# tczhangzhi/pytorch-distributed

Measured on NVIDIA H100. Metric: ResNet-50 images/sec (device-timed, max over ranks), higher is better.
Workload: dtype bf16; 1 GPU; model=resnet50, global_batch=256, image_size=224, parallelism=dp1, entry=distributed, comm=fused, nvls=False, channels_last=True, fused_bn=True, optimizer=fused, cuda_graph=True, l2_policy=inputs larger than L2 (4 x 38.5 MB bf16 batches + GBs of activations per step), overlap_optimizer=True, bucket_view=False, cudnn=deterministic

## Files before the change

### pytorch_distributed_b200/csrc/bindings.cpp

```cpp
#include <torch/extension.h>

#include "hvd_core.h"
#include "host.h"
#include "symm.h"

namespace py = pybind11;
using namespace ptd;

namespace {

at::Tensor arena_view(const std::shared_ptr<SymmArena>& a, int64_t rank, int64_t offset_bytes, int64_t numel, const std::string& dtype) {
  at::ScalarType st;
  if (dtype == "float32") st = at::kFloat;
  else if (dtype == "bfloat16") st = at::kBFloat16;
  else if (dtype == "float16") st = at::kHalf;
  else if (dtype == "int32") st = at::kInt;
  else if (dtype == "uint8") st = at::kByte;
  else throw std::runtime_error("unsupported arena view dtype " + dtype);
  const int64_t esz = (int64_t)c10::elementSize(st);
  TORCH_CHECK(offset_bytes >= 0 && offset_bytes + numel * esz <= a->bytes(), "arena view out of range");
  TORCH_CHECK(offset_bytes % esz == 0, "misaligned arena view");
  const int r = a->single_process() ? (int)rank : a->rank();
  void* p = reinterpret_cast<void*>(a->ptr(r) + offset_bytes);
  auto keep = a;
// ... 69 lines not shown
        launch_ll_allreduce(a->ctx(channel), in, out, scale, a->ll_seq_ptr());
      })
      .def("sync_bn",
           [](std::shared_ptr<SymmArena> a, int channel, int64_t xoff, int64_t calls_ptr, int as_rank) {
             TORCH_CHECK(xoff >= 0 && xoff % 16 == 0 && xoff + kSyncBnAreaBytes <= a->bytes(), "sync BN exchange area outside the arena");
             TORCH_CHECK(calls_ptr != 0, "sync BN call counters missing");
             return SyncBN{a->ctx(channel, as_rank), xoff, reinterpret_cast<uint32_t*>(calls_ptr)};
           },
           py::arg("channel"), py::arg("xoff"), py::arg("calls_ptr"), py::arg("as_rank") = 0);

  m.def("pack_pointers", &pack_pointers);
  m.def("fused_sgd_flat", &fused_sgd_flat, py::arg("grad"), py::arg("master"), py::arg("momentum"), py::arg("model_copy"), py::arg("hyper"),
        py::arg("found_inf"), py::arg("nesterov"), py::arg("first_step"));
  m.def("fused_sgd_multi", &fused_sgd_multi);
  m.def("multi_tensor_scale", &multi_tensor_scale);
  m.def("multi_tensor_axpby", &multi_tensor_axpby);
  m.def("amp_update_scale", &amp_update_scale);
  const auto sync_arg = py::arg("sync") = static_cast<const SyncBN*>(nullptr);
  m.def("bn_act_forward", &bn_act_forward, py::arg("x"), py::arg("residual"), py::arg("weight"), py::arg("bias"), py::arg("running_mean"),
        py::arg("running_var"), py::arg("num_batches_tracked"), py::arg("training"), py::arg("momentum"), py::arg("eps"), py::arg("relu"),
        py::arg("need_mask"), py::arg("work"), py::arg("stats_ready"), sync_arg);
  m.def("bn_act_backward", &bn_act_backward, py::arg("dy"), py::arg("x"), py::arg("mask"), py::arg("weight"), py::arg("saved"), py::arg("relu"),
        py::arg("has_residual"), py::arg("work"), sync_arg);
  m.def("bn_act_backward2", &bn_act_backward2, py::arg("dy_a"), py::arg("dy_b"), py::arg("x"), py::arg("mask"), py::arg("weight"),
        py::arg("saved"), py::arg("relu"), py::arg("work"), sync_arg);
  m.def("stem_forward", &stem_forward, py::arg("x"), py::arg("weight"), py::arg("bias"), py::arg("running_mean"), py::arg("running_var"),
        py::arg("num_batches_tracked"), py::arg("training"), py::arg("momentum"), py::arg("eps"), py::arg("need_code"), py::arg("work"), sync_arg);
  m.def("stem_forward_pre", &stem_forward_pre, py::arg("x"), py::arg("weight"), py::arg("bias"), py::arg("running_mean"), py::arg("running_var"),
        py::arg("num_batches_tracked"), py::arg("training"), py::arg("momentum"), py::arg("eps"), py::arg("need_code"), py::arg("work"), sync_arg);
  m.def("stem_backward", &stem_backward, py::arg("dp"), py::arg("x"), py::arg("code"), py::arg("weight"), py::arg("saved"), py::arg("work"),
        sync_arg);
  m.def("stem_im2col", &stem_im2col);
  m.def("conv1x1_bnstats", &conv1x1_bnstats, py::arg("x"), py::arg("weight"), py::arg("gsum"), sync_arg);
  m.def("normalize_nhwc", &normalize_nhwc);
  m.def("resample_normalize", &resample_normalize, py::arg("arena"), py::arg("n"), py::arg("out_h"), py::arg("out_w"), py::arg("max_rows"),
        py::arg("a"), py::arg("b"), py::arg("out_dtype"), py::arg("channels_last"));
  m.def("p2p_copy_multi", &p2p_copy_multi);

  py::class_<FusionQueue, std::shared_ptr<FusionQueue>>(m, "FusionQueue")
      .def(py::init<int64_t, double, int64_t>(), py::arg("fusion_threshold_bytes"), py::arg("cycle_time_ms"), py::arg("cycle_bytes") = 0)
      .def("wait_idle", &FusionQueue::wait_idle, py::arg("timeout_ms"), py::call_guard<py::gil_scoped_release>())
      .def("wake", &FusionQueue::wake)
      .def("set_cycle_bytes", &FusionQueue::set_cycle_bytes)
      .def("cycle_bytes", &FusionQueue::cycle_bytes)
      .def("enable_timeline", &FusionQueue::enable_timeline)
      .def("timeline", &FusionQueue::timeline)
      .def("enqueue", &FusionQueue::enqueue, py::arg("name"), py::arg("nbytes"), py::arg("order_key"))
      .def("next_group", &FusionQueue::next_group, py::arg("timeout_ms"), py::call_guard<py::gil_scoped_release>())
      .def("flush", &FusionQueue::flush)
      .def("mark_done", &FusionQueue::mark_done)
      .def("wait", &FusionQueue::wait, py::arg("handle"), py::arg("timeout_ms"), py::call_guard<py::gil_scoped_release>())
      .def("pending", &FusionQueue::pending)
      .def("shutdown", &FusionQueue::shutdown)
      .def("stats", &FusionQueue::stats);
}
```

### pytorch_distributed_b200/csrc/bn_act.cu

```cuda
#include <ATen/cuda/CUDAContext.h>
#include <c10/cuda/CUDAGuard.h>
#include <torch/extension.h>

#include <map>

#include "bn_combine.cuh"
#include "common.cuh"
#include "host.h"

namespace ptd {

constexpr int kBnThreads = 256;
constexpr int kBnWarps = kBnThreads / 32;

struct RowMap {
  int cgs;
  int tpr;
  int rpp;
  int rlocal;
  int cg0;
  bool active;
  bool pow2;
};
__device__ __forceinline__ RowMap row_map(int C) {
// ... 600 lines not shown
          float dz = to_f32<T>(from_f32<T>(d[k] + e[k]));
          if constexpr (RELU) dz = (bits >> k) & 1u ? dz : 0.f;
          d[k] = dz;
          s[k] += dz;
          q[k] += dz * (v[k] - mean[k]);
        }
        store8<T>(gout + r * C + coff, d);
      }
#pragma unroll
      for (int k = 0; k < 8; ++k) q[k] *= saved[C + cg * 8 + k];
    }
    cta_combine(m, cgb, s, q, sm, part, C);
  }
}

template <typename T>
static void bwd2_impl(const at::Tensor& dya, const at::Tensor& dyb, const at::Tensor& mask, const at::Tensor& x, const at::Tensor& saved,
                      at::Tensor& work, const at::Tensor& w, at::Tensor& g_out, at::Tensor& dx, at::Tensor& dw, at::Tensor& db, bool relu,
                      const SyncBN* sync) {
  const Geometry g = geometry(x);
  cudaStream_t st = at::cuda::getCurrentCUDAStream();
  T* gp = reinterpret_cast<T*>(g_out.data_ptr());
  const auto reduce = relu ? bn_bwd_reduce_sum_kernel<T, true> : bn_bwd_reduce_sum_kernel<T, false>;
  int rpb;
  const int rgrid = reduce_grid(g, &rpb, resident_ctas(reduce, g.smem));
  at::Tensor part = partials(x, rgrid, g.C);
  reduce<<<rgrid, kBnThreads, g.smem, st>>>(reinterpret_cast<const T*>(dya.data_ptr()), reinterpret_cast<const T*>(dyb.data_ptr()),
                                            relu ? mask.data_ptr<uint8_t>() : nullptr, reinterpret_cast<const T*>(x.data_ptr()),
                                            saved.data_ptr<float>(), gp, part.data_ptr<float>(), g.M, g.C, rpb);
  C10_CUDA_KERNEL_LAUNCH_CHECK();
  bwd_apply<T>(g, part, gp, nullptr, x, saved, work, w, dx, nullptr, dw, db, false, sync, st);
}

std::vector<at::Tensor> bn_act_backward2(const at::Tensor& dy_a_in, const at::Tensor& dy_b_in, const at::Tensor& x,
                                         const c10::optional<at::Tensor>& mask_opt, const at::Tensor& weight, const at::Tensor& saved,
                                         bool relu, at::Tensor work, const SyncBN* sync) {
  check_nhwc(x, "x");
  const auto cl = at::MemoryFormat::ChannelsLast;
  at::Tensor dya = dy_a_in.is_contiguous(cl) ? dy_a_in : dy_a_in.contiguous(cl);
  at::Tensor dyb = dy_b_in.is_contiguous(cl) ? dy_b_in : dy_b_in.contiguous(cl);
  TORCH_CHECK(dya.scalar_type() == x.scalar_type() && dya.sizes() == x.sizes() && dya.device() == x.device(), "dy_a must match x");
  TORCH_CHECK(dyb.scalar_type() == x.scalar_type() && dyb.sizes() == x.sizes() && dyb.device() == x.device(), "dy_b must match x");
  at::Tensor mask;
  if (relu) {
    TORCH_CHECK(mask_opt.has_value() && mask_opt->defined() && mask_opt->scalar_type() == at::kByte && mask_opt->numel() == x.numel() / 8,
                "ReLU backward needs the forward's bit mask");
    mask = *mask_opt;
  }
  const int C = (int)x.size(1);
  check_work(work, C, sync);
  TORCH_CHECK(saved.defined() && saved.scalar_type() == at::kFloat && saved.numel() >= 2 * C, "saved statistics missing");
  c10::cuda::CUDAGuard guard(x.device());
  at::Tensor g = at::empty_like(x, x.options().memory_format(cl));
  at::Tensor dx = at::empty_like(x, x.options().memory_format(cl));
  at::Tensor dw = at::empty_like(weight), db = at::empty_like(weight);
  for_act_dtype(x, [&](auto t) { bwd2_impl<typename decltype(t)::type>(dya, dyb, mask, x, saved, work, weight, g, dx, dw, db, relu, sync); });
  return {dx, g, dw, db};
}

}

namespace ptd {

struct PoolGeom { int H, W, OH, OW; };

__device__ __forceinline__ void stem_scale_shift(const float* gsum, const float* rm, const float* rv, const void* w, const void* b, int wdt,
// ... 433 lines not shown
```

### pytorch_distributed_b200/csrc/gemm_bnstats.cu

```cuda
#include <ATen/cuda/CUDAContext.h>
#include <c10/cuda/CUDAGuard.h>
#include <cuda.h>
#include <torch/extension.h>

#include "common.cuh"
#include "host.h"

namespace ptd {

constexpr int kBlockM = 128;
constexpr int kBlockK = 64;
constexpr int kConsumerThreads = 256;
constexpr int kGemmThreads = kConsumerThreads + 32;

template <int BLOCK_N> struct GemmCfg {
  static constexpr int kStages = BLOCK_N == 256 ? 3 : 4;
  static constexpr int kABytes = kBlockM * kBlockK * 2;
  static constexpr int kBBytes = BLOCK_N * kBlockK * 2;
  static constexpr int kCBytes = kBlockM * BLOCK_N * 2;
  static constexpr int kStatFloats = 2 * 4 * 128;
  static constexpr int kSmem = 1024 + kStages * (kABytes + kBBytes) + kCBytes + kStatFloats * 4 + 2 * kStages * 8;
};

__device__ __forceinline__ uint32_t smem_u32(const void* p) { return (uint32_t)__cvta_generic_to_shared(p); }
// ... 37 lines not shown
      "wgmma.mma_async.sync.aligned.m64n64k16.f32." TY "." TY " "                                                     \
      "{%0, %1, %2, %3, %4, %5, %6, %7, %8, %9, %10, %11, %12, %13, %14, %15, "                                       \
      "%16, %17, %18, %19, %20, %21, %22, %23, %24, %25, %26, %27, %28, %29, %30, %31}, %32, %33, p, 1, 1, 0, 0;\n\t}" \
      : PTD_F8(0), PTD_F8(8), PTD_F8(16), PTD_F8(24)                                                                  \
      : "l"(adesc), "l"(bdesc), "r"(accumulate))
#define PTD_WGMMA_N128(TY)                                                                                            \
  asm volatile(                                                                                                       \
      "{\n\t.reg .pred p;\n\tsetp.ne.b32 p, %66, 0;\n\t"                                                              \
      "wgmma.mma_async.sync.aligned.m64n128k16.f32." TY "." TY " "                                                    \
      "{%0, %1, %2, %3, %4, %5, %6, %7, %8, %9, %10, %11, %12, %13, %14, %15, "                                       \
      "%16, %17, %18, %19, %20, %21, %22, %23, %24, %25, %26, %27, %28, %29, %30, %31, "                              \
      "%32, %33, %34, %35, %36, %37, %38, %39, %40, %41, %42, %43, %44, %45, %46, %47, "                              \
      "%48, %49, %50, %51, %52, %53, %54, %55, %56, %57, %58, %59, %60, %61, %62, %63}, %64, %65, p, 1, 1, 0, 0;\n\t}" \
      : PTD_F8(0), PTD_F8(8), PTD_F8(16), PTD_F8(24), PTD_F8(32), PTD_F8(40), PTD_F8(48), PTD_F8(56)                  \
      : "l"(adesc), "l"(bdesc), "r"(accumulate))

template <typename T> __device__ __forceinline__ void wgmma_n64(float* d, uint64_t adesc, uint64_t bdesc, int accumulate) {
  if constexpr (std::is_same<T, __half>::value) PTD_WGMMA_N64("f16");
  else PTD_WGMMA_N64("bf16");
}
template <typename T> __device__ __forceinline__ void wgmma_n128(float* d, uint64_t adesc, uint64_t bdesc, int accumulate) {
  if constexpr (std::is_same<T, __half>::value) PTD_WGMMA_N128("f16");
  else PTD_WGMMA_N128("bf16");
}
#undef PTD_WGMMA_N64
#undef PTD_WGMMA_N128
#undef PTD_F8

template <int N> __device__ __forceinline__ void fence_regs(float (&d)[N]) {
#pragma unroll
  for (int i = 0; i < N; ++i) asm volatile("" : "+f"(d[i])::"memory");
}

template <typename T, int BLOCK_N>
__global__ void __launch_bounds__(kGemmThreads, 1) gemm_bnstats_kernel(const __grid_constant__ CUtensorMap tmap_a,
                                                                       const __grid_constant__ CUtensorMap tmap_b,
                                                                       const __grid_constant__ CUtensorMap tmap_c,
                                                                       float* __restrict__ part, int N, int K, int m_tiles,
                                                                       int n_tiles, int ctas_per_n) {
  using Cfg = GemmCfg<BLOCK_N>;
  constexpr int kStages = Cfg::kStages;
  constexpr int kInstN = BLOCK_N >= 128 ? 128 : 64;
  constexpr int kBoxes = BLOCK_N / 64;
  extern __shared__ uint8_t smem_raw[];
  uint8_t* smem = reinterpret_cast<uint8_t*>((reinterpret_cast<uintptr_t>(smem_raw) + 1023) & ~(uintptr_t)1023);
  uint8_t* smem_a = smem;
  uint8_t* smem_b = smem_a + kStages * Cfg::kABytes;
  uint8_t* smem_c = smem_b + kStages * Cfg::kBBytes;
  float* smem_stats = reinterpret_cast<float*>(smem_c + Cfg::kCBytes);
  uint64_t* full_bar = reinterpret_cast<uint64_t*>(smem_stats + Cfg::kStatFloats);
  uint64_t* empty_bar = full_bar + kStages;

  const int warp = threadIdx.x >> 5, lane = threadIdx.x & 31;
  const int n_tile = blockIdx.x % n_tiles;
  const int m_first = blockIdx.x / n_tiles;
  const int n0 = n_tile * BLOCK_N;
  const int num_kb = K / kBlockK;

  if (threadIdx.x == 0) {
    for (int s = 0; s < kStages; ++s) { mbar_init(&full_bar[s], 1); mbar_init(&empty_bar[s], kConsumerThreads / 32); }
    asm volatile("fence.mbarrier_init.release.cluster;" ::: "memory");
  }
  __syncthreads();

  if (warp == kConsumerThreads / 32) {
    if (lane == 0) {
      asm volatile("prefetch.tensormap [%0];" ::"l"(&tmap_a) : "memory");
      asm volatile("prefetch.tensormap [%0];" ::"l"(&tmap_b) : "memory");
      uint32_t it = 0;
      for (int mt = m_first; mt < m_tiles; mt += ctas_per_n) {
        for (int kb = 0; kb < num_kb; ++kb, ++it) {
          const int s = it % kStages;
          mbar_wait(&empty_bar[s], ((it / kStages) & 1) ^ 1);
          mbar_expect_tx(&full_bar[s], Cfg::kABytes + Cfg::kBBytes);
          tma_load_2d(smem_a + s * Cfg::kABytes, &tmap_a, &full_bar[s], kb * kBlockK, mt * kBlockM);
          tma_load_2d(smem_b + s * Cfg::kBBytes, &tmap_b, &full_bar[s], kb * kBlockK, n0);
        }
      }
    }
    return;
  }

  const int wg = warp >> 2, t = threadIdx.x & 127, w = warp & 3;
  uint8_t* stg = smem_c + wg * (Cfg::kCBytes / 2);
  float acc[BLOCK_N / 2] = {};
  const int r0 = 16 * w + (lane >> 2);
  constexpr int kPairs = BLOCK_N / 2, kParts = 128 / kPairs, kRows = 64 / kParts;
  const int p = t % kPairs, rpart = t / kPairs;
  const int p_box = p >> 5, p_gran = (p & 31) >> 2, p_byte = (p & 3) * 4;
  float s0 = 0.f, s1 = 0.f, q0 = 0.f, q1 = 0.f;

  uint32_t it = 0;
  for (int mt = m_first; mt < m_tiles; mt += ctas_per_n) {
    for (int kb = 0; kb < num_kb; ++kb, ++it) {
      const int s = it % kStages;
      mbar_wait(&full_bar[s], (it / kStages) & 1);
      const uint64_t adesc = gmma_desc(smem_a + s * Cfg::kABytes + wg * 64 * 128);
      const uint64_t bdesc = gmma_desc(smem_b + s * Cfg::kBBytes);
      fence_regs(acc);
      asm volatile("wgmma.fence.sync.aligned;" ::: "memory");
#pragma unroll
      for (int k = 0; k < kBlockK / 16; ++k) {
#pragma unroll
        for (int h = 0; h < BLOCK_N / kInstN; ++h) {
          if constexpr (kInstN == 128) wgmma_n128<T>(acc + h * 64, adesc + 2 * k, bdesc + h * 8 * kInstN + 2 * k, (kb | k) != 0);
          else wgmma_n64<T>(acc + h * 32, adesc + 2 * k, bdesc + h * 8 * kInstN + 2 * k, (kb | k) != 0);
        }
      }
      asm volatile("wgmma.commit_group.sync.aligned;" ::: "memory");
      asm volatile("wgmma.wait_group.sync.aligned 0;" ::: "memory");
      fence_regs(acc);
      if (lane == 0) mbar_arrive(&empty_bar[s]);
    }

    if (t == 0) asm volatile("cp.async.bulk.wait_group.read 0;" ::: "memory");
    named_barrier(1 + wg, 128);
#pragma unroll
    for (int j = 0; j < BLOCK_N / 8; ++j) {
      uint8_t* box = stg + (j >> 3) * 8192 + (lane & 3) * 4;
      const int g = j & 7;
      *reinterpret_cast<uint32_t*>(box + r0 * 128 + ((g ^ (r0 & 7)) << 4)) = Wire<T>::pack2(acc[4 * j], acc[4 * j + 1]);
      *reinterpret_cast<uint32_t*>(box + (r0 + 8) * 128 + ((g ^ (r0 & 7)) << 4)) =
          Wire<T>::pack2(acc[4 * j + 2], acc[4 * j + 3]);
    }
    asm volatile("fence.proxy.async.shared::cta;" ::: "memory");
    named_barrier(1 + wg, 128);
    if (t == 0) {
#pragma unroll
      for (int b = 0; b < kBoxes; ++b)
        asm volatile("cp.async.bulk.tensor.2d.global.shared::cta.bulk_group [%0, {%2, %3}], [%1];"
                     ::"l"(&tmap_c), "r"(smem_u32(stg + b * 8192)), "r"(n0 + b * 64), "r"(mt * kBlockM + wg * 64) : "memory");
      asm volatile("cp.async.bulk.commit_group;" ::: "memory");
    }
    const uint8_t* src = stg + p_box * 8192 + p_byte;
#pragma unroll 8
    for (int r = rpart * kRows; r < rpart * kRows + kRows; ++r) {
      const float2 f = Wire<T>::unpack2(*reinterpret_cast<const uint32_t*>(src + r * 128 + ((p_gran ^ (r & 7)) << 4)));
      s0 += f.x; q0 += f.x * f.x;
      s1 += f.y; q1 += f.y * f.y;
    }
  }
  if (t == 0) asm volatile("cp.async.bulk.wait_group 0;" ::: "memory");
  float* my = smem_stats + wg * 4 * 128 + t;
  my[0] = s0; my[128] = s1; my[256] = q0; my[384] = q1;
  named_barrier(3, kConsumerThreads);
  for (int i = threadIdx.x; i < 2 * BLOCK_N; i += kConsumerThreads) {
    const int half = i >= BLOCK_N, col = i - half * BLOCK_N;
    const int pair = col >> 1, which = half * 2 + (col & 1);
    float v = 0.f;
    for (int w2 = 0; w2 < 2; ++w2)
      for (int pt = 0; pt < kParts; ++pt) v += smem_stats[w2 * 4 * 128 + which * 128 + pt * kPairs + pair];
    part[(size_t)m_first * 2 * N + half * N + n0 + col] = v;
  }
}

typedef CUresult (*EncodeTiledFn)(CUtensorMap*, CUtensorMapDataType, cuuint32_t, void*, const cuuint64_t*, const cuuint64_t*, const cuuint32_t*,
                                  const cuuint32_t*, CUtensorMapInterleave, CUtensorMapSwizzle, CUtensorMapL2promotion, CUtensorMapFloatOOBfill);

static EncodeTiledFn encode_fn() {
  static EncodeTiledFn fn = nullptr;
  if (!fn) {
    void* p = nullptr;
    cudaDriverEntryPointQueryResult q;
    TORCH_CHECK(cudaGetDriverEntryPoint("cuTensorMapEncodeTiled", &p, cudaEnableDefault, &q) == cudaSuccess && p, "cuTensorMapEncodeTiled not found");
    fn = reinterpret_cast<EncodeTiledFn>(p);
  }
  return fn;
}

static CUtensorMap make_map(CUtensorMapDataType dtype, const void* ptr, int64_t rows, int64_t cols, int box_rows,
                            CUtensorMapL2promotion promo) {
  CUtensorMap m;
  cuuint64_t dims[2] = {(cuuint64_t)cols, (cuuint64_t)rows};
  cuuint64_t strides[1] = {(cuuint64_t)cols * 2};
  cuuint32_t box[2] = {(cuuint32_t)kBlockK, (cuuint32_t)box_rows};
  cuuint32_t estr[2] = {1, 1};
  CUresult r = encode_fn()(&m, dtype, 2, const_cast<void*>(ptr), dims, strides, box, estr, CU_TENSOR_MAP_INTERLEAVE_NONE,
                           CU_TENSOR_MAP_SWIZZLE_128B, promo, CU_TENSOR_MAP_FLOAT_OOB_FILL_NONE);
  TORCH_CHECK(r == CUDA_SUCCESS, "cuTensorMapEncodeTiled failed: ", (int)r);
  return m;
}

template <typename T, int BLOCK_N>
static void launch_gemm(const at::Tensor& a, const at::Tensor& b, at::Tensor& c, at::Tensor& gsum, int M, int N, int K, const SyncBN* sync) {
  constexpr int smem = GemmCfg<BLOCK_N>::kSmem;
  static bool configured[64] = {};
  const int dev = a.get_device();
  if (!configured[dev & 63]) {
    C10_CUDA_CHECK(cudaFuncSetAttribute(gemm_bnstats_kernel<T, BLOCK_N>, cudaFuncAttributeMaxDynamicSharedMemorySize, smem));
    configured[dev & 63] = true;
  }
  constexpr CUtensorMapDataType dt = std::is_same<T, __half>::value ? CU_TENSOR_MAP_DATA_TYPE_FLOAT16 : CU_TENSOR_MAP_DATA_TYPE_BFLOAT16;
  const CUtensorMap ma = make_map(dt, a.data_ptr(), M, K, kBlockM, CU_TENSOR_MAP_L2_PROMOTION_L2_256B);
  const CUtensorMap mb = make_map(dt, b.data_ptr(), N, K, BLOCK_N, CU_TENSOR_MAP_L2_PROMOTION_L2_256B);
  const CUtensorMap mc = make_map(dt, c.data_ptr(), M, N, 64, CU_TENSOR_MAP_L2_PROMOTION_NONE);
  const int m_tiles = (M + kBlockM - 1) / kBlockM, n_tiles = N / BLOCK_N;
  const int sms = at::cuda::getCurrentDeviceProperties()->multiProcessorCount;
  const int ctas_per_n = std::max(1, std::min(m_tiles, sms / n_tiles));
  const int grid = ctas_per_n * n_tiles;
  cudaStream_t st = at::cuda::getCurrentCUDAStream();
  at::Tensor part = at::empty({ctas_per_n, 2 * N}, gsum.options());
  gemm_bnstats_kernel<T, BLOCK_N><<<grid, kGemmThreads, smem, st>>>(ma, mb, mc, part.data_ptr<float>(), N, K, m_tiles, n_tiles, ctas_per_n);
  C10_CUDA_KERNEL_LAUNCH_CHECK();
  finish_sums(part.data_ptr<float>(), ctas_per_n, N, M, gsum.data_ptr<float>(), sync, st);
}

template <typename T>
static void launch_gemm_for(const at::Tensor& a, const at::Tensor& b, at::Tensor& c, at::Tensor& gsum, int M, int N, int K, const SyncBN* sync) {
  static const int max_bn = getenv("PTD_GEMM_BLOCK_N") ? atoi(getenv("PTD_GEMM_BLOCK_N")) : 256;
  if (N % 256 == 0 && max_bn >= 256) launch_gemm<T, 256>(a, b, c, gsum, M, N, K, sync);
  else if (N % 128 == 0 && max_bn >= 128) launch_gemm<T, 128>(a, b, c, gsum, M, N, K, sync);
  else launch_gemm<T, 64>(a, b, c, gsum, M, N, K, sync);
}

at::Tensor conv1x1_bnstats(const at::Tensor& x, const at::Tensor& weight, at::Tensor gsum, const SyncBN* sync) {
  const bool is16 = x.scalar_type() == at::kBFloat16 || x.scalar_type() == at::kHalf;
  TORCH_CHECK(x.is_cuda() && x.dim() == 4 && is16 && x.is_contiguous(at::MemoryFormat::ChannelsLast),
              "conv1x1_bnstats: x must be a channels_last bf16 or fp16 CUDA tensor");
  TORCH_CHECK(weight.dim() == 4 && weight.size(2) == 1 && weight.size(3) == 1 && weight.scalar_type() == x.scalar_type(),
              "conv1x1_bnstats: weight must be [N, K, 1, 1] with x's dtype (both bf16 or both fp16)");
  const int64_t M64 = x.size(0) * x.size(2) * x.size(3);
  const int K = (int)x.size(1), N = (int)weight.size(0);
  TORCH_CHECK(weight.size(1) == K && K % kBlockK == 0 && N % 64 == 0 && M64 < (int64_t)1 << 31, "conv1x1_bnstats: unsupported shape");
  check_work(gsum, N, sync);
  TORCH_CHECK((reinterpret_cast<uintptr_t>(x.data_ptr()) & 15) == 0, "x must be 16-byte aligned");
  c10::cuda::CUDAGuard guard(x.device());
  at::Tensor w2 = weight.reshape({N, K}).contiguous();
  at::Tensor y = at::empty({x.size(0), N, x.size(2), x.size(3)}, x.options().memory_format(at::MemoryFormat::ChannelsLast));
  const int M = (int)M64;
  if (x.scalar_type() == at::kHalf) launch_gemm_for<__half>(x, w2, y, gsum, M, N, K, sync);
  else launch_gemm_for<__nv_bfloat16>(x, w2, y, gsum, M, N, K, sync);
  return y;
}

}
```

### pytorch_distributed_b200/csrc/host.h

```cpp
#pragma once
#include <cuda_runtime_api.h>
#include <torch/extension.h>

#include <cstdint>
#include <string>
#include <vector>

#include "comm_types.h"

namespace ptd {

struct Seg {
  int32_t tensor;
  int32_t len;
  int64_t src_off;
  int64_t arena_off;
};
static_assert(sizeof(Seg) == 24, "Seg layout is mirrored by numpy in parallel/plan.py");

void launch_plan(const CommCtx& ctx, int kind, int wire_dtype, bool nvls, int grid, const std::vector<at::Tensor>& tensors,
                 int64_t seg_begin_ptr, int64_t segs_ptr, int64_t data_off_bytes, int64_t block_elems, int64_t plan_calls_ptr,
                 int64_t found_inf_ptr, double scale, bool writeback, int root, int flags = 0, int64_t result_off_bytes = -1);
at::Tensor pack_pointers(const std::vector<at::Tensor>& tensors);
void launch_barrier(const CommCtx& ctx);
void launch_metrics(const CommCtx& ctx, const at::Tensor& logits, const at::Tensor& target, const c10::optional<at::Tensor>& loss,
                    int64_t ll_seq_ptr, at::Tensor out);
void launch_ll_allreduce(const CommCtx& ctx, const at::Tensor& in, at::Tensor out, double scale, int64_t ll_seq_ptr);

void fused_sgd_flat(at::Tensor grad, at::Tensor master, at::Tensor momentum, c10::optional<at::Tensor> model_copy,
                    at::Tensor hyper, c10::optional<at::Tensor> found_inf, bool nesterov, bool first_step);
void fused_sgd_multi(std::vector<at::Tensor> grads, std::vector<at::Tensor> params, std::vector<at::Tensor> momenta,
                     std::vector<at::Tensor> model_copies, at::Tensor hyper, c10::optional<at::Tensor> found_inf, bool nesterov,
                     bool first_step);
void multi_tensor_scale(std::vector<at::Tensor> src, std::vector<at::Tensor> dst, double scale, at::Tensor found_inf);
void multi_tensor_axpby(std::vector<at::Tensor> x, std::vector<at::Tensor> y, std::vector<at::Tensor> out, double a, double b,
                        at::Tensor found_inf);
void amp_update_scale(at::Tensor scale, at::Tensor growth_tracker, at::Tensor found_inf, double growth, double backoff,
                      int64_t interval, at::Tensor hyper);

void combine_partials(const float* part, int nblocks, int n, float* gsum, cudaStream_t st);
std::vector<at::Tensor> bn_act_forward(const at::Tensor& x, const c10::optional<at::Tensor>& residual, const at::Tensor& weight,
                                       const at::Tensor& bias, at::Tensor running_mean, at::Tensor running_var,
                                       c10::optional<at::Tensor> num_batches_tracked, bool training, double momentum, double eps, bool relu,
                                       bool need_mask, at::Tensor work, bool stats_ready, const SyncBN* sync);
std::vector<at::Tensor> bn_act_backward(const at::Tensor& dy, const at::Tensor& x, const c10::optional<at::Tensor>& mask,
                                        const at::Tensor& weight, const at::Tensor& saved, bool relu, bool has_residual, at::Tensor work,
                                        const SyncBN* sync);
std::vector<at::Tensor> bn_act_backward2(const at::Tensor& dy_a, const at::Tensor& dy_b, const at::Tensor& x,
                                         const c10::optional<at::Tensor>& mask, const at::Tensor& weight, const at::Tensor& saved, bool relu,
                                         at::Tensor work, const SyncBN* sync);

std::vector<at::Tensor> stem_forward(const at::Tensor& x, const at::Tensor& weight, const at::Tensor& bias, at::Tensor running_mean,
                                     at::Tensor running_var, c10::optional<at::Tensor> num_batches_tracked, bool training, double momentum,
                                     double eps, bool need_code, at::Tensor work, const SyncBN* sync);
std::vector<at::Tensor> stem_forward_pre(const at::Tensor& x, const at::Tensor& weight, const at::Tensor& bias, at::Tensor running_mean,
                                         at::Tensor running_var, c10::optional<at::Tensor> num_batches_tracked, bool training, double momentum,
                                         double eps, bool need_code, at::Tensor work, const SyncBN* sync);
std::vector<at::Tensor> stem_backward(const at::Tensor& dp, const at::Tensor& x, const at::Tensor& code, const at::Tensor& weight,
                                      const at::Tensor& saved, at::Tensor work, const SyncBN* sync);

constexpr int64_t kSyncWork(int64_t C) { return 4 * C + 4; }
void sync_bn_exchange(const float* part, int nblocks, int C, int64_t rows, float* work, const SyncBN& s, cudaStream_t st);
void check_work(const at::Tensor& work, int64_t C, const SyncBN* sync);
float* work_sums(float* work, int C, const SyncBN* sync);
float* finish_sums(const float* part, int nblocks, int C, int64_t rows, float* work, const SyncBN* sync, cudaStream_t st);

at::Tensor conv1x1_bnstats(const at::Tensor& x, const at::Tensor& weight, at::Tensor gsum, const SyncBN* sync);

at::Tensor stem_im2col(const at::Tensor& x);

at::Tensor normalize_nhwc(const at::Tensor& src, const at::Tensor& mean, const at::Tensor& std, int64_t out_dtype, bool channels_last);

void p2p_copy_multi(std::vector<at::Tensor> src, std::vector<at::Tensor> dst, int64_t run_device);

at::Tensor resample_normalize(const at::Tensor& arena, int64_t n, int64_t out_h, int64_t out_w, int64_t max_rows, const at::Tensor& a,
                              const at::Tensor& b, int64_t out_dtype, bool channels_last);

}
```

### pytorch_distributed_b200/models/resnet.py

```python
from __future__ import annotations

import torch
import torch.nn as nn

from ..ops.bn_act import begin_step, bn_act
from ..ops.conv_bn import conv1x1_bn_act
from ..ops.stem import bn_relu_maxpool
from ..ops.stem_conv import can_use_stem_gemm, stem_conv_bn_relu_maxpool

import os as _os
FUSED_CONV1X1 = _os.environ.get("PTD_FUSED_CONV1X1", "1") == "1"
SPLIT_RESGRAD = _os.environ.get("PTD_SPLIT_RESGRAD", "1") == "1"
STEM_GEMM = _os.environ.get("PTD_STEM_GEMM", "1") == "1"


def _pair(x):
    return x if isinstance(x, tuple) else (x, x)


class BNAct(nn.BatchNorm2d):

    def __init__(self, num_features, relu=True, fused=None, **kw):
        super().__init__(num_features, **kw)
        self.relu = relu
        self.fused = fused

    def forward(self, x, residual=None, split=False):
        training = self.training or not self.track_running_stats
        nbt = self.num_batches_tracked if (self.training and self.track_running_stats) else None
        return bn_act(x, self.weight, self.bias, self.running_mean, self.running_var, residual=residual, relu=self.relu,
                      training=training, momentum=0.1 if self.momentum is None else self.momentum, eps=self.eps, fused=self.fused,
                      num_batches_tracked=nbt, split=split, sync=self.sync_context())

    def sync_context(self):
        return None


def check_process_group(process_group) -> None:
    import torch.distributed as dist
    if process_group is None or (dist.is_available() and dist.is_initialized() and process_group is dist.group.WORLD):
        return
    if dist.is_available() and dist.is_initialized() and dist.get_world_size(process_group) == dist.get_world_size():
        return
    raise NotImplementedError("process_group: synchronised BatchNorm over a subgroup of the ranks is not supported; "
                              "pass None (the whole world)")


class SyncBNAct(BNAct):

# ... 72 lines not shown
        super().__init__()
        if groups != 1 or base_width != 64:
            raise ValueError("BasicBlock only supports groups=1 and base_width=64")
        self.conv1 = _conv3x3(cin, planes, stride)
        self.bn1 = BNAct(planes, relu=True, fused=fused)
        self.conv2 = _conv3x3(planes, planes)
        self.bn2 = BNAct(planes, relu=True, fused=fused)
        self.downsample = downsample
        self.stride = stride

    def forward(self, x):
        x, skip = _pair(x)
        identity = skip if self.downsample is None else self.downsample(skip)
        out = self.bn1(self.conv1(x))
        return self.bn2(self.conv2(out), identity, split=SPLIT_RESGRAD and self.training)


class Bottleneck(nn.Module):
    expansion = 4

    def __init__(self, cin, planes, stride=1, downsample=None, groups=1, base_width=64, fused=None):
        super().__init__()
        width = int(planes * (base_width / 64.0)) * groups
        self.conv1 = _conv1x1(cin, width)
        self.bn1 = BNAct(width, relu=True, fused=fused)
        self.conv2 = _conv3x3(width, width, stride, groups)
        self.bn2 = BNAct(width, relu=True, fused=fused)
        self.conv3 = _conv1x1(width, planes * self.expansion)
        self.bn3 = BNAct(planes * self.expansion, relu=True, fused=fused)
        self.downsample = downsample
        self.stride = stride

    def forward(self, x):
        x, skip = _pair(x)
        identity = skip if self.downsample is None else self.downsample(skip)
        out = conv1x1_bn_act(x, self.conv1, self.bn1, enabled=FUSED_CONV1X1)
        out = self.bn2(self.conv2(out))
        return conv1x1_bn_act(out, self.conv3, self.bn3, identity, enabled=FUSED_CONV1X1, split=SPLIT_RESGRAD and self.training)


class ResNet(nn.Module):
    def __init__(self, block, layers, num_classes=1000, groups=1, width_per_group=64, fused_bn=None,
                 zero_init_residual=False):
        super().__init__()
        self.inplanes = 64
        self.groups = groups
        self.base_width = width_per_group
        self.fused_bn = fused_bn
        self.conv1 = nn.Conv2d(3, 64, 7, stride=2, padding=3, bias=False)
        self.bn1 = BNAct(64, relu=True, fused=fused_bn)
        self.maxpool = nn.MaxPool2d(3, stride=2, padding=1)
        self.layer1 = self._make_layer(block, 64, layers[0])
        self.layer2 = self._make_layer(block, 128, layers[1], stride=2)
        self.layer3 = self._make_layer(block, 256, layers[2], stride=2)
        self.layer4 = self._make_layer(block, 512, layers[3], stride=2)
        self.avgpool = nn.AdaptiveAvgPool2d((1, 1))
        self.fc = nn.Linear(512 * block.expansion, num_classes)
        for m in self.modules():
            if isinstance(m, nn.Conv2d):
                nn.init.kaiming_normal_(m.weight, mode="fan_out", nonlinearity="relu")
            elif isinstance(m, nn.BatchNorm2d):
                nn.init.constant_(m.weight, 1.0)
                nn.init.constant_(m.bias, 0.0)
        if zero_init_residual:
            for m in self.modules():
                if isinstance(m, Bottleneck):
                    nn.init.constant_(m.bn3.weight, 0.0)
                elif isinstance(m, BasicBlock):
                    nn.init.constant_(m.bn2.weight, 0.0)

    def _make_layer(self, block, planes, blocks, stride=1):
# ... 48 lines not shown
```

### pytorch_distributed_b200/ops/conv_bn.py

```python
from __future__ import annotations

import torch

from .bn_act import _BnActFn, _can_fuse, workspace
from .sync_bn import kernel_arg


class _Conv1x1Stats(torch.autograd.Function):
    @staticmethod
    def forward(ctx, x, weight, stats, sync=None):
        from .. import _ext
        _ext.note_launch(2)
        C = _ext.lib()
        y = C.conv1x1_bnstats(x, weight, stats, kernel_arg(sync, C))
        ctx.save_for_backward(x, weight)
        return y

    @staticmethod
    def backward(ctx, dy):
        x, weight = ctx.saved_tensors
        dy = dy.contiguous(memory_format=torch.channels_last)
        dx, dw, _ = torch.ops.aten.convolution_backward(dy, x, weight, None, (1, 1), (0, 0), (1, 1), False, (0, 0), 1,
                                                        (ctx.needs_input_grad[0], ctx.needs_input_grad[1], False))
        return dx, dw, None, None


GEMM_DTYPES = (torch.bfloat16, torch.float16)


def autocast_gemm_dtype():
    if torch.is_autocast_enabled("cuda"):
        dt = torch.get_autocast_dtype("cuda")
        if dt in GEMM_DTYPES:
            return dt
    return None


def gemm_weight(w, autocast_dtype):
    return w if autocast_dtype is None or w.dtype == autocast_dtype else w.to(autocast_dtype)


def can_fuse_conv1x1(x, conv) -> bool:
    w = conv.weight
    wdt = autocast_gemm_dtype() or w.dtype
    return (x.is_cuda and x.dtype in GEMM_DTYPES and wdt == x.dtype and w.is_floating_point() and x.dim() == 4
            and conv.kernel_size == (1, 1) and conv.stride == (1, 1) and conv.padding == (0, 0) and conv.groups == 1 and conv.bias is None
            and x.is_contiguous(memory_format=torch.channels_last) and x.size(1) % 64 == 0 and w.size(0) % 64 == 0
            and x.size(0) * x.size(2) * x.size(3) >= 128)


def conv1x1_bn_act(x, conv, bn, residual=None, enabled=True, split=False):
    training = bn.training or not bn.track_running_stats
    sync = bn.sync_context()
    if not (enabled and training and can_fuse_conv1x1(x, conv) and bn.fused is not False and (sync is None or sync.native is not None)):
        return bn(conv(x), residual, split) if split else bn(conv(x), residual)
    lw = workspace(x.device).layer(conv.weight.size(0), sync)
    y = _Conv1x1Stats.apply(x, gemm_weight(conv.weight, autocast_gemm_dtype()), lw.fwd, sync)
    if not _can_fuse(y, bn.weight, residual, bn.running_mean):
        return bn(y, residual, split) if split else bn(y, residual)
    need_grad = torch.is_grad_enabled() and (y.requires_grad or bn.weight.requires_grad)
    nbt = bn.num_batches_tracked if (bn.training and bn.track_running_stats) else None
    out = _BnActFn.apply(y, residual, bn.weight, bn.bias, bn.running_mean, bn.running_var, nbt, True,
                         0.1 if bn.momentum is None else float(bn.momentum), float(bn.eps), bn.relu, need_grad, lw,
                         bool(split and need_grad), sync)
    if split and not isinstance(out, tuple):
        return out, out
    return out
```

Before: 6936 images/s.

## Fuse next block's conv1 dgrad with BN-ReLU backward at bottleneck boundaries

```diff
diff --git a/pytorch_distributed_b200/csrc/bindings.cpp b/pytorch_distributed_b200/csrc/bindings.cpp
--- a/pytorch_distributed_b200/csrc/bindings.cpp
+++ b/pytorch_distributed_b200/csrc/bindings.cpp
@@ -125,6 +125,8 @@
         sync_arg);
   m.def("stem_im2col", &stem_im2col);
   m.def("conv1x1_bnstats", &conv1x1_bnstats, py::arg("x"), py::arg("weight"), py::arg("gsum"), sync_arg);
+  m.def("conv1x1_dgrad_bn_backward", &conv1x1_dgrad_bn_backward, py::arg("dy1"), py::arg("w1"), py::arg("dy_b"), py::arg("x"), py::arg("mask"),
+        py::arg("weight"), py::arg("saved"), py::arg("work"), sync_arg);
   m.def("normalize_nhwc", &normalize_nhwc);
   m.def("resample_normalize", &resample_normalize, py::arg("arena"), py::arg("n"), py::arg("out_h"), py::arg("out_w"), py::arg("max_rows"),
         py::arg("a"), py::arg("b"), py::arg("out_dtype"), py::arg("channels_last"));
diff --git a/pytorch_distributed_b200/csrc/bn_act.cu b/pytorch_distributed_b200/csrc/bn_act.cu
--- a/pytorch_distributed_b200/csrc/bn_act.cu
+++ b/pytorch_distributed_b200/csrc/bn_act.cu
@@ -656,6 +656,33 @@
   bwd_apply<T>(g, part, gp, nullptr, x, saved, work, w, dx, nullptr, dw, db, false, sync, st);
 }
 
+std::vector<at::Tensor> bn_backward_masked(const at::Tensor& g, const at::Tensor& x, const at::Tensor& weight, const at::Tensor& saved,
+                                           at::Tensor work, const SyncBN* sync) {
+  check_nhwc(x, "x");
+  check_nhwc(g, "g");
+  TORCH_CHECK(g.scalar_type() == x.scalar_type() && g.sizes() == x.sizes() && g.device() == x.device(), "g must match x");
+  const int C = (int)x.size(1);
+  check_work(work, C, sync);
+  TORCH_CHECK(saved.defined() && saved.scalar_type() == at::kFloat && saved.numel() >= 2 * C, "saved statistics missing");
+  c10::cuda::CUDAGuard guard(x.device());
+  at::Tensor dx = at::empty_like(x, x.options().memory_format(at::MemoryFormat::ChannelsLast));
+  at::Tensor dw = at::empty_like(weight), db = at::empty_like(weight);
+  for_act_dtype(x, [&](auto t) {
+    using T = typename decltype(t)::type;
+    const Geometry geo = geometry(x);
+    cudaStream_t st = at::cuda::getCurrentCUDAStream();
+    int rpb;
+    const int rgrid = reduce_grid(geo, &rpb, resident_ctas(bn_bwd_reduce_sum_kernel<T, true>, geo.smem));
+    at::Tensor part = partials(x, rgrid, C);
+    const T* gp = reinterpret_cast<const T*>(g.data_ptr());
+    bn_bwd_reduce_kernel<T, false><<<rgrid, kBnThreads, geo.smem, st>>>(gp, nullptr, reinterpret_cast<const T*>(x.data_ptr()),
+                                                                          saved.data_ptr<float>(), part.data_ptr<float>(), geo.M, C, rpb);
+    C10_CUDA_KERNEL_LAUNCH_CHECK();
+    bwd_apply<T>(geo, part, gp, nullptr, x, saved, work, weight, dx, nullptr, dw, db, false, sync, st);
+  });
+  return {dx, dw, db};
+}
+
 std::vector<at::Tensor> bn_act_backward2(const at::Tensor& dy_a_in, const at::Tensor& dy_b_in, const at::Tensor& x,
                                          const c10::optional<at::Tensor>& mask_opt, const at::Tensor& weight, const at::Tensor& saved,
                                          bool relu, at::Tensor work, const SyncBN* sync) {
diff --git a/pytorch_distributed_b200/csrc/gemm_bnstats.cu b/pytorch_distributed_b200/csrc/gemm_bnstats.cu
--- a/pytorch_distributed_b200/csrc/gemm_bnstats.cu
+++ b/pytorch_distributed_b200/csrc/gemm_bnstats.cu
@@ -93,12 +93,16 @@
   for (int i = 0; i < N; ++i) asm volatile("" : "+f"(d[i])::"memory");
 }
 
-template <typename T, int BLOCK_N>
-__global__ void __launch_bounds__(kGemmThreads, 1) gemm_bnstats_kernel(const __grid_constant__ CUtensorMap tmap_a,
-                                                                       const __grid_constant__ CUtensorMap tmap_b,
-                                                                       const __grid_constant__ CUtensorMap tmap_c,
-                                                                       float* __restrict__ part, int N, int K, int m_tiles,
-                                                                       int n_tiles, int ctas_per_n) {
+template <typename T> struct DgradEpi {
+  const T* dyb;
+  const uint8_t* mask;
+  int M;
+};
+
+template <typename T, int BLOCK_N, bool DGRAD>
+__device__ __forceinline__ void gemm_body(const CUtensorMap& tmap_a, const CUtensorMap& tmap_b, const CUtensorMap& tmap_c,
+                                          float* __restrict__ part, int N, int K, int m_tiles, int n_tiles, int ctas_per_n,
+                                          const DgradEpi<T>& e) {
   using Cfg = GemmCfg<BLOCK_N>;
   constexpr int kStages = Cfg::kStages;
   constexpr int kInstN = BLOCK_N >= 128 ? 128 : 64;
@@ -150,6 +154,8 @@
   const int p = t % kPairs, rpart = t / kPairs;
   const int p_box = p >> 5, p_gran = (p & 31) >> 2, p_byte = (p & 3) * 4;
   float s0 = 0.f, s1 = 0.f, q0 = 0.f, q1 = 0.f;
+  constexpr int kGran = BLOCK_N / 8, kGParts = 128 / kGran, kGRows = 64 / kGParts, kU = BLOCK_N == 256 ? 8 : 4;
+  const int gc = t % kGran, gpart = t / kGran;
 
   uint32_t it = 0;
   for (int mt = m_first; mt < m_tiles; mt += ctas_per_n) {
@@ -184,6 +190,47 @@
       *reinterpret_cast<uint32_t*>(box + (r0 + 8) * 128 + ((g ^ (r0 & 7)) << 4)) =
           Wire<T>::pack2(acc[4 * j + 2], acc[4 * j + 3]);
     }
+    if constexpr (DGRAD) {
+#pragma unroll
+      for (int i = 0; i < BLOCK_N / 2; ++i) acc[i] = 0.f;
+      named_barrier(1 + wg, 128);
+      const int row0 = mt * kBlockM + wg * 64, col = n0 + gc * 8;
+      uint8_t* gcol = stg + (gc >> 3) * 8192;
+      const int gsl = gc & 7;
+#pragma unroll 1
+      for (int rb = gpart * kGRows; rb < gpart * kGRows + kGRows; rb += kU) {
+        V4 b[kU];
+        uint32_t bits[kU];
+#pragma unroll
+        for (int u = 0; u < kU; ++u) {
+          const int row = row0 + rb + u;
+          if (row < e.M) {
+            b[u] = ld_stream(e.dyb + (size_t)row * N + col);
+            bits[u] = e.mask[(size_t)row * (N >> 3) + (col >> 3)];
+          } else {
+            b[u] = V4{0u, 0u, 0u, 0u};
+            bits[u] = 0u;
+          }
+        }
+#pragma unroll
+        for (int u = 0; u < kU; ++u) {
+          const int r = rb + u;
+          V4* slot = reinterpret_cast<V4*>(gcol + r * 128 + ((gsl ^ (r & 7)) << 4));
+          const V4 a = *slot;
+          const uint32_t aw[4] = {a.x, a.y, a.z, a.w}, bw[4] = {b[u].x, b[u].y, b[u].z, b[u].w};
+          uint32_t gw[4];
+#pragma unroll
+          for (int h = 0; h < 4; ++h) {
+            const float2 fa = Wire<T>::unpack2(aw[h]), fb = Wire<T>::unpack2(bw[h]);
+            float g0 = to_f32<T>(from_f32<T>(fa.x + fb.x)), g1 = to_f32<T>(from_f32<T>(fa.y + fb.y));
+            g0 = (bits[u] >> (2 * h)) & 1u ? g0 : 0.f;
+            g1 = (bits[u] >> (2 * h + 1)) & 1u ? g1 : 0.f;
+            gw[h] = Wire<T>::pack2(g0, g1);
+          }
+          *slot = V4{gw[0], gw[1], gw[2], gw[3]};
+        }
+      }
+    }
     asm volatile("fence.proxy.async.shared::cta;" ::: "memory");
     named_barrier(1 + wg, 128);
     if (t == 0) {
@@ -193,15 +240,18 @@
                      ::"l"(&tmap_c), "r"(smem_u32(stg + b * 8192)), "r"(n0 + b * 64), "r"(mt * kBlockM + wg * 64) : "memory");
       asm volatile("cp.async.bulk.commit_group;" ::: "memory");
     }
-    const uint8_t* src = stg + p_box * 8192 + p_byte;
+    if constexpr (!DGRAD) {
+      const uint8_t* src = stg + p_box * 8192 + p_byte;
 #pragma unroll 8
-    for (int r = rpart * kRows; r < rpart * kRows + kRows; ++r) {
-      const float2 f = Wire<T>::unpack2(*reinterpret_cast<const uint32_t*>(src + r * 128 + ((p_gran ^ (r & 7)) << 4)));
-      s0 += f.x; q0 += f.x * f.x;
-      s1 += f.y; q1 += f.y * f.y;
+      for (int r = rpart * kRows; r < rpart * kRows + kRows; ++r) {
+        const float2 f = Wire<T>::unpack2(*reinterpret_cast<const uint32_t*>(src + r * 128 + ((p_gran ^ (r & 7)) << 4)));
+        s0 += f.x; q0 += f.x * f.x;
+        s1 += f.y; q1 += f.y * f.y;
+      }
     }
   }
   if (t == 0) asm volatile("cp.async.bulk.wait_group 0;" ::: "memory");
+  if constexpr (DGRAD) return;
   float* my = smem_stats + wg * 4 * 128 + t;
   my[0] = s0; my[128] = s1; my[256] = q0; my[384] = q1;
   named_barrier(3, kConsumerThreads);
@@ -213,6 +263,24 @@
       for (int pt = 0; pt < kParts; ++pt) v += smem_stats[w2 * 4 * 128 + which * 128 + pt * kPairs + pair];
     part[(size_t)m_first * 2 * N + half * N + n0 + col] = v;
   }
+}
+
+template <typename T, int BLOCK_N>
+__global__ void __launch_bounds__(kGemmThreads, 1) gemm_bnstats_kernel(const __grid_constant__ CUtensorMap tmap_a,
+                                                                       const __grid_constant__ CUtensorMap tmap_b,
+                                                                       const __grid_constant__ CUtensorMap tmap_c,
+                                                                       float* __restrict__ part, int N, int K, int m_tiles,
+                                                                       int n_tiles, int ctas_per_n) {
+  gemm_body<T, BLOCK_N, false>(tmap_a, tmap_b, tmap_c, part, N, K, m_tiles, n_tiles, ctas_per_n, DgradEpi<T>{});
+}
+
+template <typename T, int BLOCK_N>
+__global__ void __launch_bounds__(kGemmThreads, 1) gemm_dgrad_bnbwd_kernel(const __grid_constant__ CUtensorMap tmap_a,
+                                                                           const __grid_constant__ CUtensorMap tmap_b,
+                                                                           const __grid_constant__ CUtensorMap tmap_c,
+                                                                           int N, int K, int m_tiles, int n_tiles, int ctas_per_n,
+                                                                           const DgradEpi<T> e) {
+  gemm_body<T, BLOCK_N, true>(tmap_a, tmap_b, tmap_c, nullptr, N, K, m_tiles, n_tiles, ctas_per_n, e);
 }
 
 typedef CUresult (*EncodeTiledFn)(CUtensorMap*, CUtensorMapDataType, cuuint32_t, void*, const cuuint64_t*, const cuuint64_t*, const cuuint32_t*,
@@ -243,13 +311,14 @@
 }
 
 template <typename T, int BLOCK_N>
-static void launch_gemm(const at::Tensor& a, const at::Tensor& b, at::Tensor& c, at::Tensor& gsum, int M, int N, int K, const SyncBN* sync) {
+static at::Tensor launch_gemm(const at::Tensor& a, const at::Tensor& b, at::Tensor& c, int M, int N, int K, const DgradEpi<T>* dg) {
   constexpr int smem = GemmCfg<BLOCK_N>::kSmem;
-  static bool configured[64] = {};
+  static bool configured[2][64] = {};
   const int dev = a.get_device();
-  if (!configured[dev & 63]) {
-    C10_CUDA_CHECK(cudaFuncSetAttribute(gemm_bnstats_kernel<T, BLOCK_N>, cudaFuncAttributeMaxDynamicSharedMemorySize, smem));
-    configured[dev & 63] = true;
+  if (!configured[dg != nullptr][dev & 63]) {
+    if (dg) C10_CUDA_CHECK(cudaFuncSetAttribute(gemm_dgrad_bnbwd_kernel<T, BLOCK_N>, cudaFuncAttributeMaxDynamicSharedMemorySize, smem));
+    else C10_CUDA_CHECK(cudaFuncSetAttribute(gemm_bnstats_kernel<T, BLOCK_N>, cudaFuncAttributeMaxDynamicSharedMemorySize, smem));
+    configured[dg != nullptr][dev & 63] = true;
   }
   constexpr CUtensorMapDataType dt = std::is_same<T, __half>::value ? CU_TENSOR_MAP_DATA_TYPE_FLOAT16 : CU_TENSOR_MAP_DATA_TYPE_BFLOAT16;
   const CUtensorMap ma = make_map(dt, a.data_ptr(), M, K, kBlockM, CU_TENSOR_MAP_L2_PROMOTION_L2_256B);
@@ -260,18 +329,24 @@
   const int ctas_per_n = std::max(1, std::min(m_tiles, sms / n_tiles));
   const int grid = ctas_per_n * n_tiles;
   cudaStream_t st = at::cuda::getCurrentCUDAStream();
-  at::Tensor part = at::empty({ctas_per_n, 2 * N}, gsum.options());
-  gemm_bnstats_kernel<T, BLOCK_N><<<grid, kGemmThreads, smem, st>>>(ma, mb, mc, part.data_ptr<float>(), N, K, m_tiles, n_tiles, ctas_per_n);
+  at::Tensor part;
+  if (dg) {
+    gemm_dgrad_bnbwd_kernel<T, BLOCK_N><<<grid, kGemmThreads, smem, st>>>(ma, mb, mc, N, K, m_tiles, n_tiles, ctas_per_n, *dg);
+  } else {
+    part = at::empty({ctas_per_n, 2 * N}, a.options().dtype(at::kFloat).memory_format(at::MemoryFormat::Contiguous));
+    gemm_bnstats_kernel<T, BLOCK_N><<<grid, kGemmThreads, smem, st>>>(ma, mb, mc, part.data_ptr<float>(), N, K, m_tiles, n_tiles, ctas_per_n);
+  }
   C10_CUDA_KERNEL_LAUNCH_CHECK();
-  finish_sums(part.data_ptr<float>(), ctas_per_n, N, M, gsum.data_ptr<float>(), sync, st);
+  return part;
 }
 
 template <typename T>
-static void launch_gemm_for(const at::Tensor& a, const at::Tensor& b, at::Tensor& c, at::Tensor& gsum, int M, int N, int K, const SyncBN* sync) {
+static at::Tensor launch_gemm_for(const at::Tensor& a, const at::Tensor& b, at::Tensor& c, int M, int N, int K,
+                                  const DgradEpi<T>* dg = nullptr) {
   static const int max_bn = getenv("PTD_GEMM_BLOCK_N") ? atoi(getenv("PTD_GEMM_BLOCK_N")) : 256;
-  if (N % 256 == 0 && max_bn >= 256) launch_gemm<T, 256>(a, b, c, gsum, M, N, K, sync);
-  else if (N % 128 == 0 && max_bn >= 128) launch_gemm<T, 128>(a, b, c, gsum, M, N, K, sync);
-  else launch_gemm<T, 64>(a, b, c, gsum, M, N, K, sync);
+  if (N % 256 == 0 && max_bn >= 256) return launch_gemm<T, 256>(a, b, c, M, N, K, dg);
+  if (N % 128 == 0 && max_bn >= 128) return launch_gemm<T, 128>(a, b, c, M, N, K, dg);
+  return launch_gemm<T, 64>(a, b, c, M, N, K, dg);
 }
 
 at::Tensor conv1x1_bnstats(const at::Tensor& x, const at::Tensor& weight, at::Tensor gsum, const SyncBN* sync) {
@@ -289,9 +364,45 @@
   at::Tensor w2 = weight.reshape({N, K}).contiguous();
   at::Tensor y = at::empty({x.size(0), N, x.size(2), x.size(3)}, x.options().memory_format(at::MemoryFormat::ChannelsLast));
   const int M = (int)M64;
-  if (x.scalar_type() == at::kHalf) launch_gemm_for<__half>(x, w2, y, gsum, M, N, K, sync);
-  else launch_gemm_for<__nv_bfloat16>(x, w2, y, gsum, M, N, K, sync);
+  at::Tensor part = x.scalar_type() == at::kHalf ? launch_gemm_for<__half>(x, w2, y, M, N, K) : launch_gemm_for<__nv_bfloat16>(x, w2, y, M, N, K);
+  finish_sums(part.data_ptr<float>(), (int)part.size(0), N, M, gsum.data_ptr<float>(), sync, at::cuda::getCurrentCUDAStream());
   return y;
 }
 
-}
+std::vector<at::Tensor> conv1x1_dgrad_bn_backward(const at::Tensor& dy1, const at::Tensor& w1, const at::Tensor& dyb_in, const at::Tensor& x,
+                                                  const at::Tensor& mask, const at::Tensor& weight, const at::Tensor& saved, at::Tensor work,
+                                                  const SyncBN* sync) {
+  const auto cl = at::MemoryFormat::ChannelsLast;
+  const bool is16 = x.scalar_type() == at::kBFloat16 || x.scalar_type() == at::kHalf;
+  TORCH_CHECK(x.is_cuda() && x.dim() == 4 && is16 && x.is_contiguous(cl), "conv1x1_dgrad_bn_backward: x must be a channels_last bf16 or fp16 CUDA tensor");
+  TORCH_CHECK(dy1.is_contiguous(cl) && dy1.scalar_type() == x.scalar_type() && dy1.dim() == 4 && dy1.size(0) == x.size(0) &&
+              dy1.size(2) == x.size(2) && dy1.size(3) == x.size(3) && dy1.device() == x.device(),
+              "conv1x1_dgrad_bn_backward: dy1 must be a channels_last tensor of x's dtype and spatial shape");
+  const int64_t M64 = x.size(0) * x.size(2) * x.size(3);
+  const int N = (int)x.size(1), K = (int)dy1.size(1);
+  TORCH_CHECK(w1.dim() == 4 && w1.size(0) == K && w1.size(1) == N && w1.size(2) == 1 && w1.size(3) == 1 && w1.scalar_type() == x.scalar_type(),
+              "conv1x1_dgrad_bn_backward: w1 must be [dy1 channels, x channels, 1, 1] of x's dtype");
+  TORCH_CHECK(K % kBlockK == 0 && N % 64 == 0 && M64 < (int64_t)1 << 31, "conv1x1_dgrad_bn_backward: unsupported shape");
+  at::Tensor dyb = dyb_in.is_contiguous(cl) ? dyb_in : dyb_in.contiguous(cl);
+  TORCH_CHECK(dyb.scalar_type() == x.scalar_type() && dyb.sizes() == x.sizes() && dyb.device() == x.device(), "dy_b must match x");
+  TORCH_CHECK(mask.is_contiguous() && mask.scalar_type() == at::kByte && mask.numel() == x.numel() / 8, "ReLU backward needs the forward's bit mask");
+  TORCH_CHECK(saved.is_contiguous() && saved.scalar_type() == at::kFloat && saved.numel() >= 2 * N, "saved statistics missing");
+  check_work(work, N, sync);
+  TORCH_CHECK(((reinterpret_cast<uintptr_t>(dy1.data_ptr()) | reinterpret_cast<uintptr_t>(dyb.data_ptr())) & 15) == 0,
+              "conv1x1_dgrad_bn_backward: dy1 and dy_b must be 16-byte aligned");
+  c10::cuda::CUDAGuard guard(x.device());
+  at::Tensor b = w1.reshape({K, N}).t().contiguous();
+  at::Tensor g = at::empty_like(x, x.options().memory_format(cl));
+  const int M = (int)M64;
+  if (x.scalar_type() == at::kHalf) {
+    const DgradEpi<__half> e{reinterpret_cast<const __half*>(dyb.data_ptr()), mask.data_ptr<uint8_t>(), M};
+    launch_gemm_for<__half>(dy1, b, g, M, N, K, &e);
+  } else {
+    const DgradEpi<__nv_bfloat16> e{reinterpret_cast<const __nv_bfloat16*>(dyb.data_ptr()), mask.data_ptr<uint8_t>(), M};
+    launch_gemm_for<__nv_bfloat16>(dy1, b, g, M, N, K, &e);
+  }
+  std::vector<at::Tensor> r = bn_backward_masked(g, x, weight, saved, work, sync);
+  return {r[0], g, r[1], r[2]};
+}
+
+}
diff --git a/pytorch_distributed_b200/csrc/host.h b/pytorch_distributed_b200/csrc/host.h
--- a/pytorch_distributed_b200/csrc/host.h
+++ b/pytorch_distributed_b200/csrc/host.h
@@ -49,6 +49,8 @@
 std::vector<at::Tensor> bn_act_backward2(const at::Tensor& dy_a, const at::Tensor& dy_b, const at::Tensor& x,
                                          const c10::optional<at::Tensor>& mask, const at::Tensor& weight, const at::Tensor& saved, bool relu,
                                          at::Tensor work, const SyncBN* sync);
+std::vector<at::Tensor> bn_backward_masked(const at::Tensor& g, const at::Tensor& x, const at::Tensor& weight, const at::Tensor& saved,
+                                           at::Tensor work, const SyncBN* sync);
 
 std::vector<at::Tensor> stem_forward(const at::Tensor& x, const at::Tensor& weight, const at::Tensor& bias, at::Tensor running_mean,
                                      at::Tensor running_var, c10::optional<at::Tensor> num_batches_tracked, bool training, double momentum,
@@ -66,6 +68,9 @@
 float* finish_sums(const float* part, int nblocks, int C, int64_t rows, float* work, const SyncBN* sync, cudaStream_t st);
 
 at::Tensor conv1x1_bnstats(const at::Tensor& x, const at::Tensor& weight, at::Tensor gsum, const SyncBN* sync);
+std::vector<at::Tensor> conv1x1_dgrad_bn_backward(const at::Tensor& dy1, const at::Tensor& w1, const at::Tensor& dy_b, const at::Tensor& x,
+                                                  const at::Tensor& mask, const at::Tensor& weight, const at::Tensor& saved, at::Tensor work,
+                                                  const SyncBN* sync);
 
 at::Tensor stem_im2col(const at::Tensor& x);
 
diff --git a/pytorch_distributed_b200/models/resnet.py b/pytorch_distributed_b200/models/resnet.py
--- a/pytorch_distributed_b200/models/resnet.py
+++ b/pytorch_distributed_b200/models/resnet.py
@@ -4,7 +4,7 @@
 import torch.nn as nn
 
 from ..ops.bn_act import begin_step, bn_act
-from ..ops.conv_bn import conv1x1_bn_act
+from ..ops.conv_bn import PendingBN, boundary_conv1x1_bn_act, conv1x1_bn_act
 from ..ops.stem import bn_relu_maxpool
 from ..ops.stem_conv import can_use_stem_gemm, stem_conv_bn_relu_maxpool
 
@@ -15,6 +15,8 @@
 
 
 def _pair(x):
+    if isinstance(x, PendingBN):
+        return x.materialize()
     return x if isinstance(x, tuple) else (x, x)
 
 
@@ -153,11 +155,16 @@
         self.stride = stride
 
     def forward(self, x):
-        x, skip = _pair(x)
-        identity = skip if self.downsample is None else self.downsample(skip)
-        out = conv1x1_bn_act(x, self.conv1, self.bn1, enabled=FUSED_CONV1X1)
+        if isinstance(x, PendingBN):
+            skip, out = boundary_conv1x1_bn_act(x, self.conv1, self.bn1, enabled=FUSED_CONV1X1)
+            identity = skip if self.downsample is None else self.downsample(skip)
+        else:
+            x, skip = _pair(x)
+            identity = skip if self.downsample is None else self.downsample(skip)
+            out = conv1x1_bn_act(x, self.conv1, self.bn1, enabled=FUSED_CONV1X1)
         out = self.bn2(self.conv2(out))
-        return conv1x1_bn_act(out, self.conv3, self.bn3, identity, enabled=FUSED_CONV1X1, split=SPLIT_RESGRAD and self.training)
+        return conv1x1_bn_act(out, self.conv3, self.bn3, identity, enabled=FUSED_CONV1X1, split=SPLIT_RESGRAD and self.training,
+                              defer=True)
 
 
 class ResNet(nn.Module):
diff --git a/pytorch_distributed_b200/ops/conv_bn.py b/pytorch_distributed_b200/ops/conv_bn.py
--- a/pytorch_distributed_b200/ops/conv_bn.py
+++ b/pytorch_distributed_b200/ops/conv_bn.py
@@ -49,7 +49,7 @@
             and x.size(0) * x.size(2) * x.size(3) >= 128)
 
 
-def conv1x1_bn_act(x, conv, bn, residual=None, enabled=True, split=False):
+def conv1x1_bn_act(x, conv, bn, residual=None, enabled=True, split=False, defer=False):
     training = bn.training or not bn.track_running_stats
     sync = bn.sync_context()
     if not (enabled and training and can_fuse_conv1x1(x, conv) and bn.fused is not False and (sync is None or sync.native is not None)):
@@ -59,10 +59,70 @@
     if not _can_fuse(y, bn.weight, residual, bn.running_mean):
         return bn(y, residual, split) if split else bn(y, residual)
     need_grad = torch.is_grad_enabled() and (y.requires_grad or bn.weight.requires_grad)
+    if defer and split and need_grad and bn.relu:
+        return PendingBN(y, residual, bn, lw, sync)
+    return _bn_apply(y, residual, bn, lw, bool(split and need_grad), sync, need_grad)
+
+
+def _bn_apply(y, residual, bn, lw, split, sync, need_grad):
     nbt = bn.num_batches_tracked if (bn.training and bn.track_running_stats) else None
     out = _BnActFn.apply(y, residual, bn.weight, bn.bias, bn.running_mean, bn.running_var, nbt, True,
-                         0.1 if bn.momentum is None else float(bn.momentum), float(bn.eps), bn.relu, need_grad, lw,
-                         bool(split and need_grad), sync)
+                         0.1 if bn.momentum is None else float(bn.momentum), float(bn.eps), bn.relu, need_grad, lw, split, sync)
     if split and not isinstance(out, tuple):
         return out, out
     return out
+
+
+class PendingBN:
+
+    __slots__ = ("y", "identity", "bn", "lw", "sync")
+
+    def __init__(self, y, identity, bn, lw, sync):
+        self.y, self.identity, self.bn, self.lw, self.sync = y, identity, bn, lw, sync
+
+    def materialize(self):
+        return _bn_apply(self.y, self.identity, self.bn, self.lw, True, self.sync, True)
+
+
+class _BoundaryFn(torch.autograd.Function):
+
+    @staticmethod
+    def forward(ctx, y, identity, weight, bias, w1, running_mean, running_var, nbt, momentum, eps, lw, sync, lw1, sync1):
+        from .. import _ext
+        C = _ext.lib()
+        _ext.note_launch(3)
+        z, saved, mask = C.bn_act_forward(y, identity, weight, bias, running_mean, running_var, nbt, True, momentum, eps, True, True,
+                                          lw.fwd, True, kernel_arg(sync, C))
+        y1 = C.conv1x1_bnstats(z, w1, lw1.fwd, kernel_arg(sync1, C))
+        ctx.save_for_backward(y, mask, weight, saved, z, w1)
+        ctx.sync, ctx.work = sync, lw
+        return z, y1
+
+    @staticmethod
+    def backward(ctx, dz, dy1):
+        from .. import _ext
+        y, mask, weight, saved, z, w1 = ctx.saved_tensors
+        C = _ext.lib()
+        cl = torch.channels_last
+        dy1 = dy1.contiguous(memory_format=cl)
+        _ext.note_launch(3)
+        dy, g, dw, db = C.conv1x1_dgrad_bn_backward(dy1, w1, dz.contiguous(memory_format=cl), y, mask, weight, saved, ctx.work.bwd(),
+                                                    kernel_arg(ctx.sync, C))
+        dw1 = torch.ops.aten.convolution_backward(dy1, z, w1, None, (1, 1), (0, 0), (1, 1), False, (0, 0), 1, (False, True, False))[1]
+        return (dy, g, dw, db, dw1) + (None,) * 9
+
+
+def boundary_conv1x1_bn_act(p: PendingBN, conv, bn, enabled=True):
+    training = bn.training or not bn.track_running_stats
+    sync1 = bn.sync_context()
+    if not (enabled and training and can_fuse_conv1x1(p.y, conv) and bn.fused is not False and (sync1 is None or sync1.native is not None)):
+        x, skip = p.materialize()
+        return skip, conv1x1_bn_act(x, conv, bn, enabled=enabled)
+    lw1 = workspace(p.y.device).layer(conv.weight.size(0), sync1)
+    b3 = p.bn
+    nbt = b3.num_batches_tracked if (b3.training and b3.track_running_stats) else None
+    z, y1 = _BoundaryFn.apply(p.y, p.identity, b3.weight, b3.bias, gemm_weight(conv.weight, autocast_gemm_dtype()), b3.running_mean,
+                              b3.running_var, nbt, 0.1 if b3.momentum is None else float(b3.momentum), float(b3.eps), p.lw, p.sync, lw1,
+                              sync1)
+    need_grad = torch.is_grad_enabled() and (y1.requires_grad or bn.weight.requires_grad)
+    return z, _bn_apply(y1, None, bn, lw1, False, sync1, need_grad)
```

After: 7068 images/s, median of 6. +1.9%, better.
